# ictnlp/StreamSpeech

Measured on NVIDIA H100. Metric: audio-seconds/sec (RTF^-1) Fr-En simul S2ST @chunk=320ms, higher is better.
Workload: dtype f32

## Files before the change

### include/streamspeech_b200.h

```cpp
#ifndef STREAMSPEECH_B200_H_
#define STREAMSPEECH_B200_H_

#include <stdint.h>

#ifdef __cplusplus
extern "C" {
#endif

typedef struct ss_engine ss_engine;

enum ss_status {
  SS_OK = 0,
  SS_ERR_INVALID = -1,
  SS_ERR_MISSING = -2,
  SS_ERR_CUDA = -3,
  SS_ERR_STATE = -4,
  SS_ERR_CAPACITY = -5
};

#define SS_MAX_UPS 8
#define SS_MAX_RB 4
#define SS_MAX_DIL 4

typedef struct ss_config {
// ... 63 lines not shown
                        float* wav_out_dev);
int ss_vocoder_hop(const ss_engine* h);
int ss_vocoder_receptive_field(const ss_engine* h);

int ss_pool_create(ss_engine* h, int n_slots, int max_seconds);
int ss_pool_create_rate(ss_engine* h, int n_slots, int max_seconds, int sample_rate);
int ss_pool_reset(ss_engine* h, int slot);
int ss_pool_push_audio(ss_engine* h, void* stream, int slot, const float* samples_host, int n);
int ss_pool_finish(ss_engine* h, int slot);
int ss_pool_info(ss_engine* h, int slot, int64_t* n_audio, int32_t* n_feat, int32_t* T_final, float** enc_out_dev, float** feats_dev);
int ss_pool_step(ss_engine* h, void* stream, int n, const int32_t* slots_host, int ctc_heads, int64_t* packed_out_dev, int64_t packed_capacity,
                 int32_t* T_out_host, int32_t* T_final_out_host, int64_t* out_off_host);

int ss_op_linear(ss_engine* h, void* stream, const float* x_dev, int M, int K, const float* w_dev, const float* bias_dev, int N,
                 int act, float* out_dev);
int ss_op_linear_umma(ss_engine* h, void* stream, const float* x_dev, int M, int K, const float* w_dev, const float* bias_dev, int N,
                      int act, int pieces, float* out_dev);
int ss_op_conv1d(ss_engine* h, void* stream, const float* x_dev, int L, int C_in, const float* w_dev, const float* bias_dev, int N,
                 int ksize, int dil, int pad_left, float pre_lrelu, int mode, float* out_dev);
int ss_set_option(ss_engine* h, const char* name, int value);
int ss_debug_copy(ss_engine* h, const char* what, void* host_dst, size_t bytes);
int ss_op_layer_norm(ss_engine* h, void* stream, const float* x_dev, int rows, int C, const float* g_dev, const float* b_dev,
                     float* out_dev);

int64_t ss_launch_count(const ss_engine* h);
int ss_async_error(ss_engine* h);

#ifdef __cplusplus
}
#endif
#endif
```

### streamspeech_b200/csrc/engine.h

```cpp
#pragma once
#include <cuda_runtime.h>

#include <map>
#include <tuple>
#include <utility>
#include <string>
#include <vector>

#include "../../include/streamspeech_b200.h"
#include "kernels.h"
#include "kernels_persist.h"
#include "kernels_multistream.h"

namespace ss {

struct HostTensor {
  std::vector<float> data;
  std::vector<int64_t> shape;
  int64_t numel() const {
    int64_t n = 1;
    for (auto s : shape) n *= s;
    return n;
  }
};
// ... 43 lines not shown
  float* bias = nullptr;
};

struct Arena {
  char* base = nullptr;
  size_t cap = 0, off = 0;
  float* f32(size_t n) { return (float*)raw(n * 4); }
  void* raw(size_t bytes);
  void reset() { off = 0; }
  bool ensure(size_t bytes);
};

}

struct ss_engine {
  int device = 0;
  ss_config cfg{};
  std::string err;
  bool finalized = false;
  int attn_chunk = 8, conv_chunk = 8;
  int umma_vocoder = 0;
  int umma_linear = 0;
  int unit_grouped = 1;
  int umma_min_rows = 128;
  int umma_min_channels = 16;
  ss::Umma2Cache* umma2_cache = nullptr;
  int vocoder_streams = 1;
  cudaStream_t aux_stream[2] = {nullptr, nullptr};
  cudaEvent_t fork_event = nullptr, join_event[2] = {nullptr, nullptr};
  int vocoder_graph = 0;
  int graph_pdl = 0;
  cudaStream_t capture_stream = nullptr;
  std::map<std::tuple<int, uintptr_t, int, int, int>, std::pair<cudaGraphExec_t, int>> voc_graphs;
  int vocoder_fused = -1;
  std::map<std::pair<int, uintptr_t>, ss::VocFusedParams> voc_fused;
  float* persist_ffn_scratch = nullptr;
  float* cl_blobs = nullptr;
  int cluster_cooperative = 1;
  long long cl_steps = 0;
  int persistent_encoder_cluster = 0;
  int persistent_ffn_fused = 1;
  int fbank_tma = 1;
  int persistent_encoder = 1;
  std::map<std::string, ss::HostTensor> host;
  std::vector<void*> dev_allocs;

// ... 103 lines not shown
```

### streamspeech_b200/csrc/engine_run.cu

```cuda
#include <algorithm>
#include <cmath>
#include <cstring>
#include <stdexcept>
#include <tuple>

#include "engine.h"

using namespace ss;

namespace {

inline cudaStream_t S(void* s) { return (cudaStream_t)s; }

int check_launch(ss_engine* h, const char* where) {
  cudaError_t e = cudaGetLastError();
  if (e != cudaSuccess) return h->fail(SS_ERR_CUDA, std::string(where) + ": " + cudaGetErrorString(e));
  return SS_OK;
}

thread_local int g_umma_linear = 0;
thread_local int g_umma_conv = 0;
thread_local int g_umma_min_rows = 128;
thread_local int g_umma_min_channels = 16;
thread_local Umma2Cache* g_umma2_cache = nullptr;
// ... 180 lines not shown
        const float s = m + 1 < nd ? 1.0f : 1.0f / nrb;
        job(rbT[j], nullptr, nullptr, L, L, ch, w2.ksize, 1, (w2.ksize - 1) / 2, 0.1f, w2.lin.w, w2.lin.b, out, ch, 1, 0, cur, s, s);
      }
      phase(first);
    }
  }
  if (!ok || jobs.size() > VOC_MAX_JOBS || phases.size() > VOC_MAX_PHASES || vocoder_fused_smem(a_stride, b_stride) > 200 * 1024) return nullptr;
  if (h->voc_fused.size() >= 64) h->voc_fused.clear();
  VocFusedParams& p = h->voc_fused[key];
  std::copy(jobs.begin(), jobs.end(), p.jobs);
  std::copy(phases.begin(), phases.end(), p.phases);
  p.n_phases = (int)phases.size();
  p.a_stride = a_stride;
  p.b_stride = b_stride;
  return &p;
}

struct DecScratch {
  float *y, *q, *kv, *attn, *hid, *qkv;
};

void dec_layer(const DecLayerW& L, float* x, int n, int dim, int ffn, int heads, bool causal, int self_kv_len_limit,
               const int* self_kv_len_dev, float* cache_k, float* cache_v, int past, const float* cross_kv, int Tk,
               const int* cross_len_dev, DecScratch& s, cudaStream_t st, int group_R = 0, const int* group_len_dev = nullptr) {
  const float scale = 0.125f;
  if (group_R > 1 && !cache_k && causal && n % group_R == 0) {
    const int S = n / group_R;
    ln_linear(x, dim * group_R, S, L.self_ln, L.qkv, ep_out(s.qkv, 3 * dim), s.y, st);
    grouped_causal_attention(s.qkv, 3 * dim, s.qkv + dim, 3 * dim, s.qkv + 2 * dim, 3 * dim, s.attn, dim, S, group_R, heads, scale, group_len_dev, st);
  } else if (cache_k) {
    ln_qkv_routed(x, dim, n, L.self_ln, L.qkv, dim, s.q, dim, cache_k + (size_t)past * dim, dim, cache_v + (size_t)past * dim, dim, s.y, st);
    mha_attention(s.q, dim, cache_k, dim, cache_v, dim, s.attn, dim, 1, n, past + n, heads, scale, 1, past, self_kv_len_dev, st);
  } else {
    ln_linear(x, dim, n, L.self_ln, L.qkv, ep_out(s.qkv, 3 * dim), s.y, st);
    mha_attention(s.qkv, 3 * dim, s.qkv + dim, 3 * dim, s.qkv + 2 * dim, 3 * dim, s.attn, dim, 1, n, n, heads, scale,
                  causal ? 1 : 0, 0, self_kv_len_dev, st);
  }
  (void)self_kv_len_limit;
  linear(s.attn, dim, n, L.out, ep_residual(x, dim), st);
  if (L.has_cross) {
    ln_linear(x, dim, n, L.cross_ln, L.cq, ep_out(s.q, dim), s.y, st);
    mha_attention(s.q, dim, cross_kv, 2 * dim, cross_kv + dim, 2 * dim, s.attn, dim, 1, n, Tk, heads, scale, 0, 0, cross_len_dev, st);
    linear(s.attn, dim, n, L.cout, ep_residual(x, dim), st);
  }
  ln_linear(x, dim, n, L.final_ln, L.fc1, ep_out(s.hid, ffn, ACT_RELU), s.y, st);
  linear(s.hid, ffn, n, L.fc2, ep_residual(x, dim), st);
}

int ensure_mt_cross(ss_engine* h, int T, int keep_rows = 0) {
  if (T <= h->mt_cross_cap) return SS_OK;
  const int cap = std::max(T + T / 2, 512);
  const size_t row = (size_t)2 * h->cfg.mt_dim;
  float* fresh = nullptr;
  if (cudaMalloc((void**)&fresh, (size_t)h->cfg.mt_layers * cap * row * sizeof(float)) != cudaSuccess) return h->fail(SS_ERR_CUDA, "cudaMalloc(mt cross kv) failed");
  if (h->mt_cross_kv) {
    cudaDeviceSynchronize();
    if (keep_rows > 0)
      for (int l = 0; l < h->cfg.mt_layers; ++l)
        cudaMemcpy(fresh + (size_t)l * cap * row, h->mt_cross_kv + (size_t)l * h->mt_cross_cap * row, (size_t)keep_rows * row * sizeof(float), cudaMemcpyDeviceToDevice);
// ... 636 lines not shown
  float* t2u = t2u_out_dev ? t2u_out_dev : h->ws.f32((size_t)Slen * dim);
  int* kvlen = nullptr;
  int* kvlen_up = nullptr;
  if (n_pad_tail > 0) {
    int v[2] = {Slen - n_pad_tail, (Slen - n_pad_tail) * R};
    kvlen = (int*)h->ws.raw(2 * sizeof(int));
    kvlen_up = kvlen + 1;
    cudaMemcpyAsync(kvlen, v, sizeof(v), cudaMemcpyHostToDevice, st);
    cudaStreamSynchronize(st);
  }
  copy_f32(mt_feats_dev, x, (int64_t)Slen * dim, st);
  for (int l = 0; l < c.t2u_layers; ++l)
    dec_layer(h->t2u[l], x, Slen, dim, c.unit_ffn, c.unit_heads, c.uni_encoder != 0, 0, kvlen, nullptr, nullptr, 0, nullptr, 0, nullptr, s1, st);
  layer_norm(x, dim, t2u, dim, h->t2u_ln.g, h->t2u_ln.b, Slen, dim, st);
  DecScratch s2 = dec_scratch(h, L, dim, c.unit_ffn);
  float* xu = h->ws.f32((size_t)L * dim);
  float* ckv = h->ws.f32((size_t)Slen * 2 * dim);
  float* logits = logits_dev ? logits_dev : h->ws.f32((size_t)L * c.unit_vocab);
  if (!xu || !ckv || !logits) return h->fail(SS_ERR_CUDA, "workspace too small");
  repeat_rows_add(t2u, Slen, R, dim, h->unit_pos_row, xu, st);
  for (int l = 0; l < c.unit_layers; ++l) {
    linear(t2u, dim, Slen, h->unit[l].ckv, ep_out(ckv, 2 * dim), st);
    const int gR = (l == 0 && h->unit_grouped) ? R : 0;
    dec_layer(h->unit[l], xu, L, dim, c.unit_ffn, c.unit_heads, true, 0, kvlen_up, nullptr, nullptr, 0, ckv, Slen, kvlen, s2, st, gR, kvlen);
  }
  layer_norm(xu, dim, xu, dim, h->unit_ln.g, h->unit_ln.b, L, dim, st);
  Linear outp;
  outp.w = h->unit_emb; outp.b = nullptr; outp.N = c.unit_vocab; outp.K = dim;
  linear(xu, dim, L, outp, ep_out(logits, c.unit_vocab), st);
  argmax_rows(logits, c.unit_vocab, L, c.unit_vocab, h->mask_pad_unk, mask_eos ? 3 : 2, argmax_dev, nullptr, st);
  ctc_collapse(argmax_dev, L, c.unit_vocab - 1, c.pad, units_dev, nullptr, count_dev, st);
  return check_launch(h, "ss_t2u_unit_decode");
}

int ss_unit_position_row(ss_engine* h, const float* row_host) {
  if (!h || !h->finalized || !row_host) return h ? h->fail(SS_ERR_STATE, "engine not finalized / null row") : SS_ERR_INVALID;
  cudaDeviceSynchronize();
  if (cudaMemcpy(h->unit_pos_row, row_host, (size_t)h->cfg.unit_dim * sizeof(float), cudaMemcpyHostToDevice) != cudaSuccess)
    return h->fail(SS_ERR_CUDA, "cudaMemcpy(unit positional row) failed");
  return SS_OK;
}

int ss_vocoder_durations(ss_engine* h, void* stream, const int64_t* codes_dev, int U, int dur_prediction, int64_t* dur_out_dev,
                         int32_t* cumsum_out_dev) {
  if (!h || !h->finalized) return h ? h->fail(SS_ERR_STATE, "engine not finalized") : SS_ERR_INVALID;
  if (!h->has_vocoder) return h->fail(SS_ERR_STATE, "no vocoder weights were loaded");
  if (U <= 0) return h->fail(SS_ERR_INVALID, "empty code sequence");
// ... 239 lines not shown
  if (n == "umma_vocoder") h->umma_vocoder = value;
  else if (n == "umma_linear") h->umma_linear = value;
  else if (n == "umma_min_rows") h->umma_min_rows = value;
  else if (n == "umma_min_channels") h->umma_min_channels = value;
  else if (n == "umma2_cache_clear") {
    umma2_cache_clear(h->umma2_cache);
    clear_graphs(h);
  }
  else if (n == "umma2_split_below") { g_umma2_split_below = value; clear_graphs(h); }
  else if (n == "umma2_min_units") { g_umma2_min_units = value; clear_graphs(h); }
  else if (n == "umma2_debug") {
    if (value && !g_umma2_dbg) {
      if (cudaMalloc(&g_umma2_dbg, 16 * sizeof(unsigned long long)) != cudaSuccess) return h->fail(SS_ERR_CUDA, "cudaMalloc failed");
      cudaMemset(g_umma2_dbg, 0, 16 * sizeof(unsigned long long));
    }
    if (!value && g_umma2_dbg) {
      cudaDeviceSynchronize();
      cudaFree(g_umma2_dbg);
      g_umma2_dbg = nullptr;
    }
  }
  else if (n == "prefer_shared") g_prefer_shared = value;
  else if (n == "unit_grouped") h->unit_grouped = value;
  else if (n == "vocoder_graph") h->vocoder_graph = value;
  else if (n == "vocoder_fused") h->vocoder_fused = value;
  else if (n == "graph_pdl") h->graph_pdl = value;
  else if (n == "fbank_tma") h->fbank_tma = value;
  else if (n == "umma2_fused_reduce") g_umma2_fused_reduce = value;
  else if (n == "persistent_encoder") h->persistent_encoder = value;
  else if (n == "persistent_ffn_fused") h->persistent_ffn_fused = value;
  else if (n == "cluster_cooperative") h->cluster_cooperative = value;
  else if (n == "persistent_encoder_cluster") {
    if (value && !h->cl_blobs) {
      if (!h->persist_layers || !h->persist_bar) return h->fail(SS_ERR_STATE, "persistent_encoder_cluster needs a finalized engine");
      const size_t n_f = encoder_layers_cluster_blob_floats(h->cfg.enc_layers);
      if (h->cfg.enc_dim != 256 || h->cfg.enc_ffn != 2048) return h->fail(SS_ERR_INVALID, "persistent_encoder_cluster: encoder must be 256 / 2048");
      if (cudaMalloc(&h->cl_blobs, n_f * sizeof(float)) != cudaSuccess) return h->fail(SS_ERR_CUDA, "cudaMalloc failed");
      h->dev_allocs.push_back(h->cl_blobs);
      encoder_layers_cluster_pack(h->persist_layers, h->cfg.enc_layers, h->cfg.dw_kernel, h->cl_blobs, 0);
      if (cudaDeviceSynchronize() != cudaSuccess) return h->fail(SS_ERR_CUDA, "packing the cluster weight blobs failed");
    }
    h->persistent_encoder_cluster = value;
  }
  else if (n == "vocoder_streams") h->vocoder_streams = value;
  else if (n == "persistent_mt") h->persistent_mt = value;
  else if (n == "persistent_mt_prefix") h->persistent_mt_prefix = value;
// ... 118 lines not shown
  } else if (mode >= 2) {
    return h->fail(SS_ERR_INVALID, "modes 2 / 3 (first-generation tensor-core kernel) were removed: use 12 / 13");
  } else {
    gemm_conv(a, w_dev, N, ep, S(stream));
  }
  return check_launch(h, "ss_op_conv1d");
}

int ss_op_linear(ss_engine* h, void* stream, const float* x_dev, int M, int K, const float* w_dev, const float* bias_dev, int N, int act,
                 float* out_dev) {
  if (!h) return SS_ERR_INVALID;
  Linear l;
  l.w = const_cast<float*>(w_dev); l.b = const_cast<float*>(bias_dev); l.N = N; l.K = K;
  linear(x_dev, K, M, l, ep_out(out_dev, N, act), S(stream));
  return check_launch(h, "ss_op_linear");
}

int ss_op_layer_norm(ss_engine* h, void* stream, const float* x_dev, int rows, int C, const float* g_dev, const float* b_dev, float* out_dev) {
  if (!h) return SS_ERR_INVALID;
  layer_norm(x_dev, C, out_dev, C, g_dev, b_dev, rows, C, S(stream));
  return check_launch(h, "ss_op_layer_norm");
}

}

#include "engine_pool.inc"
```

### streamspeech_b200/csrc/kernels.h

```cpp
#pragma once
#include <cuda_runtime.h>
#include <stdint.h>

namespace ss {

extern unsigned long long g_launches;
extern int g_prefer_shared;
extern thread_local int g_pdl_off;

enum Act : int { ACT_NONE = 0, ACT_RELU = 1, ACT_SILU = 2, ACT_TANH = 3 };

struct ConvA {
  const float* x = nullptr;
  int B = 1;
  int L_in = 0;
  int L_rows = 0;
  int C_in = 0;
  int ldx = 0;
  int ksize = 1;
  int stride = 1;
  int dil = 1;
  int pad_left = 0;
  int chunk = 0;
  float pre_lrelu = 1.0f;
// ... 78 lines not shown
int vocoder_fused(const VocFusedParams& p, unsigned* bar_ctr, unsigned* bar_target_host, cudaStream_t st);

bool skinny_gemm_supported(int M, int N, int K, const Epilogue& ep);
void skinny_gemm(const float* A, int lda, const float* W, int M, int N, int K, const Epilogue& ep, cudaStream_t st);

void layer_norm(const float* x, int ldx, float* y, int ldy, const float* gamma, const float* beta, int rows, int C,
                cudaStream_t st);

void fbank_cmvn(const float* samples, int64_t n_samples, int f0, int nf, const float* mel_bank ,
                const float* window , const float* cmvn_mean, const float* cmvn_inv_std_or_null,
                const float* cmvn_std, float* out , cudaStream_t st);

void fbank_cmvn_tma(const float* samples, int f0, int nf, const float* melT, const float* window, const float* cmvn_mean, const float* cmvn_std,
                    float* out, cudaStream_t st);

void relpos_attention(const float* q, int ldq, const float* k, int ldk, const float* v, int ldv, const float* pos, int Tpos,
                      const float* bias_u, const float* bias_v, float* out, int B, int nQ, int q_offset, int T, int H, int D,
                      int chunk , const int* lengths_dev, cudaStream_t st);

void mha_attention(const float* q, int ldq, const float* k, int ldk, const float* v, int ldv, float* out, int ldo, int B,
                   int Tq, int Tk, int H, float scale, int causal, int causal_offset, const int* kv_len_dev,
                   cudaStream_t st);

void grouped_causal_attention(const float* q, int ldq, const float* k, int ldk, const float* v, int ldv, float* out, int ldo, int S, int R,
                              int H, float scale, const int* kv_len_dev, cudaStream_t st);

void depthwise_bn_silu(const float* x, int ldx, const float* w , const float* scale, const float* shift,
                       float* y, int ldy, int B, int T, int t0, int n, int C, int k, int chunk, cudaStream_t st);

void scale_rows(float* x, int64_t n, float s, cudaStream_t st);
void embed_tokens_pos(const int64_t* tokens, const int* positions_or_null, int pos_offset, const float* emb,
                      const float* pos_table, float scale, float* out, int rows, int C, int pad_idx, cudaStream_t st);
void repeat_rows_add(const float* x, int S, int R, int C, const float* addvec_or_null, float* out, cudaStream_t st);
void argmax_rows(const float* logits, int ld, int rows, int V, const int* masked_cols, int n_masked, int64_t* out_idx,
                 float* out_lprob_or_null, cudaStream_t st);
void ctc_collapse(const int64_t* argmax, int n, int blank, int pad, int64_t* out_tokens, int* out_index, int* out_count,
                  cudaStream_t st);
void ctc_argmax_collapse_pair(const float* logits, int ld, int V, int n_new, int row0, int n_rows, const int* masked, int n_masked, int blank,
                              int pad, int64_t* am0, int64_t* am1, int64_t* out, int out_stride, unsigned* ticket, cudaStream_t st);
void gather_rows(const int64_t* idx, int n, int idx_offset, const float* table, int C, float* out, cudaStream_t st);
void duration_from_log(const float* logdur, int n, int64_t* dur, int* cumsum , cudaStream_t st);
void expand_frames(const float* emb , const int* cumsum , int U, int f0, int nf, int C, float* out,
                   cudaStream_t st);
void conv_post_tanh(const float* x, int L, int C, const float* w , float bias, int k, float pre_slope, float* out,
                    cudaStream_t st);
void copy_f32(const float* src, float* dst, int64_t n, cudaStream_t st);
// ... 5 lines not shown
```

### streamspeech_b200/csrc/kernels_attn.cu

```cuda
#include "common.cuh"
#include "kernels.h"

namespace ss {
namespace {

constexpr int QT = 16;
constexpr int KT = 64;
constexpr int ATT_NT = 128;
constexpr int HD = 64;
constexpr int LDK = HD + 4;

__device__ __forceinline__ float dot64(const float* __restrict__ a, const float* __restrict__ b) {
  float acc = 0.f;
#pragma unroll
  for (int d = 0; d < HD; d += 4) {
    float4 x = *reinterpret_cast<const float4*>(a + d);
    float4 y = *reinterpret_cast<const float4*>(b + d);
    acc = fmaf(x.x, y.x, acc);
    acc = fmaf(x.y, y.y, acc);
    acc = fmaf(x.z, y.z, acc);
    acc = fmaf(x.w, y.w, acc);
  }
  return acc;
}
// ... 262 lines not shown
    float e = expf(smem[j] - mx);
    smem[j] = e;
    if (j < n_prev) sum += e;
  }
  sum = block_sum128(sum, red);
  __syncthreads();
  {
    const int d = threadIdx.x & (HD - 1), half = threadIdx.x >> 6;
    float a = 0.f;
    for (int j = half; j < n_prev; j += 2) a = fmaf(smem[j], v[(int64_t)j * ldv + h * HD + d], a);
    part[half][d] = a;
  }
  __syncthreads();
  const float e_own = own ? smem[n_prev] : 0.f;
  for (int idx = threadIdx.x; idx < R * HD; idx += ATT_NT) {
    const int r = idx >> 6, d = idx & (HD - 1);
    const float c = own ? (float)(r + 1) : 0.f;
    const float num = (float)R * (part[0][d] + part[1][d]) + c * e_own * (own ? v[(int64_t)g * ldv + h * HD + d] : 0.f);
    const float den = (float)R * sum + c * e_own;
    out[((int64_t)g * R + r) * ldo + h * HD + d] = num / den;
  }
}

template <bool RELPOS>
void launch_attn(const float* q, int ldq, const float* k, int ldk, const float* v, int ldv, const float* pos, int Tpos, int ldp,
                 const float* bias_u, const float* bias_v, float* out, int ldo, int B, int nQ, int q_offset, int T, int H, float scale,
                 int chunk, int causal, int causal_offset, const int* lengths, cudaStream_t st) {
  const long tiles = (long)((nQ + QT - 1) / QT) * H * B;
  if (tiles < 96 && (size_t)T * sizeof(float) <= 160 * 1024) {
    size_t smem_row = (size_t)((T + 3) & ~3) * sizeof(float);
    if (smem_row > 40 * 1024 && first_time_on_device((const void*)attn_row_kernel<RELPOS>))
      cudaFuncSetAttribute(attn_row_kernel<RELPOS>, cudaFuncAttributeMaxDynamicSharedMemorySize, 160 * 1024);
    launch_pdl(attn_row_kernel<RELPOS>, dim3(dim3(nQ, H, B)), dim3(ATT_NT), smem_row, st, q, ldq, k, ldk, v, ldv, pos, Tpos, ldp, bias_u, bias_v, out, ldo, nQ,
                                                                      q_offset, T, scale, chunk, causal, causal_offset, lengths);
    return;
  }
  size_t smem = (size_t)((RELPOS ? 2 : 1) * QT * LDK + 2 * KT * LDK + (RELPOS ? (KT + QT - 1) * LDK : 0) + QT * (KT + 1)) * sizeof(float);
  if (first_time_on_device((const void*)attn_tile_kernel<RELPOS>))
    cudaFuncSetAttribute(attn_tile_kernel<RELPOS>, cudaFuncAttributeMaxDynamicSharedMemorySize, (int)smem);
  launch_pdl(attn_tile_kernel<RELPOS>, dim3(dim3((nQ + QT - 1) / QT, H, B)), dim3(ATT_NT), smem, st, q, ldq, k, ldk, v, ldv, pos, Tpos, ldp, bias_u, bias_v, out, ldo,
                                                                                 nQ, q_offset, T, scale, chunk, causal, causal_offset, lengths);
}

}

void relpos_attention(const float* q, int ldq, const float* k, int ldk, const float* v, int ldv, const float* pos, int Tpos,
                      const float* bias_u, const float* bias_v, float* out, int B, int nQ, int q_offset, int T, int H, int D,
                      int chunk, const int* lengths_dev, cudaStream_t st) {
  ++g_launches;
  if (B <= 0 || T <= 0 || nQ <= 0) return;
  launch_attn<true>(q, ldq, k, ldk, v, ldv, pos, Tpos, D, bias_u, bias_v, out, D, B, nQ, q_offset, T, H, 0.125f, chunk, 0, 0, lengths_dev, st);
}

void grouped_causal_attention(const float* q, int ldq, const float* k, int ldk, const float* v, int ldv, float* out, int ldo, int S, int R,
                              int H, float scale, const int* kv_len_dev, cudaStream_t st) {
  ++g_launches;
  if (S <= 0 || R <= 0) return;
  launch_pdl(grouped_causal_attn_kernel, dim3(S, H), dim3(ATT_NT), (size_t)((S + 3) & ~3) * sizeof(float), st, q, ldq, k, ldk, v, ldv, out, ldo, S, R,
             scale, kv_len_dev);
}

void mha_attention(const float* q, int ldq, const float* k, int ldk, const float* v, int ldv, float* out, int ldo, int B,
                   int Tq, int Tk, int H, float scale, int causal, int causal_offset, const int* kv_len_dev,
                   cudaStream_t st) {
  ++g_launches;
  if (B <= 0 || Tq <= 0 || Tk <= 0) return;
  launch_attn<false>(q, ldq, k, ldk, v, ldv, nullptr, 0, 0, nullptr, nullptr, out, ldo, B, Tq, 0, Tk, H, scale, 0, causal, causal_offset,
                     kv_len_dev, st);
}

}
```

### streamspeech_b200/engine.py

```python
from __future__ import annotations

import ctypes
import os
from typing import Dict, List, Optional, Sequence, Tuple

import torch

from . import constants
from .config import ModelConfig

_HERE = os.path.dirname(os.path.abspath(__file__))
LIB_PATH = os.path.join(_HERE, "libstreamspeech_b200.so")
SS_MAX_UPS, SS_MAX_RB, SS_MAX_DIL = 8, 4, 4


class SSConfig(ctypes.Structure):
    _fields_ = (
        [(n, ctypes.c_int32) for n in (
            "feat_dim", "enc_dim", "enc_ffn", "enc_heads", "enc_layers", "dw_kernel", "conv_channels", "conv_kernel",
            "src_vocab", "tgt_vocab", "mt_dim", "mt_ffn", "mt_heads", "mt_layers",
            "t2u_layers", "unit_dim", "unit_ffn", "unit_heads", "unit_layers", "unit_vocab", "ctc_upsample_rate",
            "bos", "pad", "eos", "unk", "uni_encoder", "max_enc_frames", "max_mt_positions", "voc_n_ups")]
        + [("voc_up_rates", ctypes.c_int32 * SS_MAX_UPS), ("voc_up_kernels", ctypes.c_int32 * SS_MAX_UPS),
           ("voc_init_channels", ctypes.c_int32), ("voc_n_rb", ctypes.c_int32),
# ... 34 lines not shown
    lib.ss_fbank.argtypes = [vp, vp, vp, i64, i64, i64, vp]
    lib.ss_encoder_forward.argtypes = [vp, vp, vp, vp, i32, i32, vp]
    lib.ss_encoder_stream_reset.argtypes = [vp]
    lib.ss_encoder_stream_step.argtypes = [vp, vp, vp, i32, vp, ctypes.POINTER(i32), ctypes.POINTER(i32)]
    lib.ss_ctc_greedy.argtypes = [vp, vp, i32, vp, i32, vp, vp, vp, vp]
    lib.ss_ctc_greedy_rows.argtypes = [vp, vp, i32, vp, i32, i32, vp, vp, vp, vp]
    lib.ss_ctc_greedy_pair.argtypes = [vp, vp, vp, i32, i32, vp, vp, vp]
    lib.ss_mt_greedy.argtypes = [vp, vp, vp, i32, vp, i32, i32, i32, vp, i32, ctypes.POINTER(i32), vp]
    lib.ss_mt_stable_rows.argtypes = [vp, i32]
    lib.ss_mt_incremental_reset.argtypes = [vp]
    lib.ss_mt_greedy_incremental.argtypes = [vp, vp, vp, i32, vp, i32, i32, i32, vp, i32, ctypes.POINTER(i32)]
    lib.ss_mt_features.argtypes = [vp, vp, vp, i32, vp, i32, vp, vp]
    lib.ss_t2u_unit_decode.argtypes = [vp, vp, vp, i32, i32, i32, vp, vp, vp, vp, vp]
    lib.ss_unit_position_row.argtypes = [vp, vp]
    lib.ss_vocoder_durations.argtypes = [vp, vp, vp, i32, i32, vp, vp]
    lib.ss_vocoder_generate.argtypes = [vp, vp, i32, i32, i32, i32, vp]
    lib.ss_vocoder_hop.argtypes = [vp]
    lib.ss_vocoder_receptive_field.argtypes = [vp]
    lib.ss_op_linear.argtypes = [vp, vp, vp, i32, i32, vp, vp, i32, i32, vp]
    lib.ss_op_linear_umma.argtypes = [vp, vp, vp, i32, i32, vp, vp, i32, i32, i32, vp]
    lib.ss_op_conv1d.argtypes = [vp, vp, vp, i32, i32, vp, vp, i32, i32, i32, i32, ctypes.c_float, i32, vp]
    lib.ss_set_option.argtypes = [vp, ctypes.c_char_p, i32]
    lib.ss_op_layer_norm.argtypes = [vp, vp, vp, i32, i32, vp, vp, vp]
    lib.ss_debug_copy.argtypes = [vp, ctypes.c_char_p, vp, ctypes.c_size_t]
    lib.ss_launch_count.argtypes = [vp]
    lib.ss_launch_count.restype = i64
    lib.ss_async_error.argtypes = [vp]
    lib.ss_resample_out_len.argtypes = [i64, i32]
    lib.ss_resample_out_len.restype = i64
    lib.ss_resample_48k_to_16k.argtypes = [vp, vp, vp, i64, i64, i64, vp]
    lib.ss_pool_create.argtypes = [vp, i32, i32]
    lib.ss_pool_create_rate.argtypes = [vp, i32, i32, i32]
    lib.ss_pool_reset.argtypes = [vp, i32]
    lib.ss_pool_finish.argtypes = [vp, i32]
    lib.ss_pool_push_audio.argtypes = [vp, vp, i32, vp, i32]
    lib.ss_pool_info.argtypes = [vp, i32, ctypes.POINTER(i64), ctypes.POINTER(i32), ctypes.POINTER(i32), ctypes.POINTER(vp), ctypes.POINTER(vp)]
    lib.ss_pool_step.argtypes = [vp, vp, i32, vp, i32, vp, i64, vp, vp, vp]
    _lib = lib
    return lib


EXPORTED_SYMBOLS = [
    "ss_create", "ss_destroy", "ss_last_error", "ss_version", "ss_load_tensor", "ss_finalize", "ss_set_chunk",
    "ss_fbank_num_frames", "ss_fbank", "ss_encoder_out_frames", "ss_encoder_forward", "ss_encoder_stream_reset", "ss_encoder_stream_step", "ss_ctc_greedy", "ss_ctc_greedy_rows", "ss_mt_greedy",
    "ss_mt_features", "ss_mt_stable_rows", "ss_t2u_unit_decode", "ss_unit_position_row", "ss_vocoder_durations", "ss_vocoder_generate", "ss_vocoder_hop",
    "ss_vocoder_receptive_field", "ss_op_linear", "ss_op_linear_umma", "ss_op_conv1d", "ss_set_option", "ss_debug_copy", "ss_op_layer_norm", "ss_launch_count", "ss_async_error", "ss_mt_incremental_reset", "ss_mt_greedy_incremental", "ss_ctc_greedy_pair", "ss_resample_out_len", "ss_resample_48k_to_16k", "ss_pool_create", "ss_pool_reset", "ss_pool_push_audio", "ss_pool_info", "ss_pool_step",
    "ss_pool_create_rate", "ss_pool_finish",
]


def make_ss_config(cfg: ModelConfig, max_enc_frames: int, max_mt_positions: int = 1024) -> SSConfig:
    c = SSConfig()
    for n in ("feat_dim", "enc_dim", "enc_ffn", "enc_heads", "enc_layers", "dw_kernel", "conv_channels", "conv_kernel",
              "src_vocab", "tgt_vocab", "mt_dim", "mt_ffn", "mt_heads", "mt_layers", "t2u_layers", "unit_dim", "unit_ffn",
              "unit_heads", "unit_layers", "unit_vocab", "ctc_upsample_rate", "bos", "pad", "eos", "unk"):
        setattr(c, n, int(getattr(cfg, n)))
    c.uni_encoder = int(cfg.uni_encoder)
    c.max_enc_frames = max_enc_frames
    c.max_mt_positions = max_mt_positions
    v = cfg.vocoder
    c.voc_n_ups = len(v.upsample_rates)
    for i, (u, k) in enumerate(zip(v.upsample_rates, v.upsample_kernel_sizes)):
        c.voc_up_rates[i], c.voc_up_kernels[i] = u, k
    c.voc_init_channels = v.upsample_initial_channel
    c.voc_n_rb = len(v.resblock_kernel_sizes)
    c.voc_rb_ndil = len(v.resblock_dilation_sizes[0])
    for j, (k, dils) in enumerate(zip(v.resblock_kernel_sizes, v.resblock_dilation_sizes)):
        c.voc_rb_kernels[j] = k
        assert len(dils) == c.voc_rb_ndil
        for m, d in enumerate(dils):
# ... 46 lines not shown
            if gcmvn is not None:
                self._load("__const__.gcmvn_mean", torch.as_tensor(gcmvn["mean"], dtype=torch.float32))
                self._load("__const__.gcmvn_std", torch.as_tensor(gcmvn["std"], dtype=torch.float32))
            self._check(self.lib.ss_finalize(self._h))
        except Exception:
            self.close()
            raise
        self.set_option("prefer_shared", int(os.environ.get("SS_PREFER_SHARED", "0")))
        self.set_option("umma_vocoder", int(os.environ.get("SS_UMMA_VOCODER", "12")))
        self.set_option("umma_linear", int(os.environ.get("SS_UMMA_LINEAR", "13")))
        self.set_option("umma_min_rows", int(os.environ.get("SS_UMMA_MIN_ROWS", "128")))
        self.set_option("umma_min_channels", int(os.environ.get("SS_UMMA_MIN_CHANNELS", "16")))
        self.set_option("persistent_encoder", int(os.environ.get("SS_PERSISTENT_ENCODER", "1")))
        self.set_option("persistent_mt", int(os.environ.get("SS_PERSISTENT_MT", "1")))
        self.set_option("umma2_fused_reduce", int(os.environ.get("SS_UMMA2_FUSED_REDUCE", "0")))
        self.set_option("fbank_tma", int(os.environ.get("SS_FBANK_TMA", "1")))
        self.set_option("persistent_ffn_fused", int(os.environ.get("SS_PERSISTENT_FFN_FUSED", "1")))
        self.set_option("persistent_encoder_cluster", int(os.environ.get("SS_PERSISTENT_ENCODER_CLUSTER", "1")))
        self.set_option("cluster_cooperative", int(os.environ.get("SS_CLUSTER_COOPERATIVE", "1")))
        self.set_option("persistent_mt_v2", int(os.environ.get("SS_PERSISTENT_MT_V2", "1")))
        self.set_option("persistent_mt_prefix", int(os.environ.get("SS_PERSISTENT_MT_PREFIX", "1")))
        self.set_option("vocoder_streams", int(os.environ.get("SS_VOCODER_STREAMS", "1")))
        self.set_option("unit_grouped", int(os.environ.get("SS_UNIT_GROUPED", "1")))
        self.set_option("vocoder_graph", int(os.environ.get("SS_VOCODER_GRAPH", "0")))
        self.set_option("vocoder_fused", int(os.environ.get("SS_VOCODER_FUSED", "-1")))
        self.set_option("graph_pdl", int(os.environ.get("SS_GRAPH_PDL", "0")))
        self.set_option("persistent_prefetch", int(os.environ.get("SS_PERSISTENT_PREFETCH", "0")))
        self.set_option("umma2_split_below", int(os.environ.get("SS_UMMA2_SPLIT_BELOW", "60")))
        self.set_option("umma2_min_units", int(os.environ.get("SS_UMMA2_MIN_UNITS", "4")))
        self.set_option("persistent_barrier", int(os.environ.get("SS_PERSISTENT_BARRIER", "1")))
        self.hop = self.lib.ss_vocoder_hop(self._h)
        self.vocoder_receptive_field = self.lib.ss_vocoder_receptive_field(self._h)

    def close(self):
        if getattr(self, "_h", None) is not None and self._h:
            self.lib.ss_destroy(self._h)
            self._h = None

    def __del__(self):
        try:
            self.close()
        except Exception:
            pass

    def _check(self, rc: int):
        if rc != 0:
# ... 270 lines not shown
        sl = (ctypes.c_int32 * n)(*[int(x) for x in slots])
        T, Tf, off = (ctypes.c_int32 * n)(), (ctypes.c_int32 * n)(), (ctypes.c_int64 * n)()
        self._check(self.lib.ss_pool_step(self._h, self._stream(), n, sl, int(ctc_heads), self._pool_out.data_ptr(), self._pool_out.numel(), T, Tf, off))
        res = [{"T": int(T[i]), "T_final": int(Tf[i]), "ctc": []} for i in range(n)]
        if ctc_heads:
            used = int(off[n - 1]) + ctc_heads * (2 * int(T[n - 1]) + 2)
            host = self._pool_out[:used].cpu()
            for i in range(n):
                Ti = int(T[i])
                for hd in range(ctc_heads):
                    o = int(off[i]) + hd * (2 * Ti + 2)
                    row = host[o:o + 2 * Ti + 2]
                    cnt = int(row[:1].view(torch.int32)[0])
                    res[i]["ctc"].append((row[1:1 + cnt].tolist(), row[1 + Ti:].view(torch.int32)[:cnt].tolist()))
        return res

    def set_option(self, name: str, value: int):
        self._check(self.lib.ss_set_option(self._h, name.encode(), int(value)))

    def op_layer_norm(self, x: torch.Tensor, g: torch.Tensor, b: torch.Tensor) -> torch.Tensor:
        out = torch.empty_like(x)
        self._check(self.lib.ss_op_layer_norm(self._h, self._stream(), x.data_ptr(), x.shape[0], x.shape[1], g.data_ptr(), b.data_ptr(), out.data_ptr()))
        return out
```

Baseline: 133.0.

## Add tensor-core flash causal attention for unit decoder self-attention

Adds a flash-style causal self-attention kernel built on bf16 mma.sync. It splits each fp32 value into three bf16 parts and runs six products per tile, so accuracy stays close to fp32. The kernel is used in the unit decoder's non-grouped layers behind a new option that is on by default, replacing the scalar mha_attention path. It also exposes a standalone op for testing. The three-way split roughly multiplies tensor-core work and adds conversion overhead in exchange for using the MMA units instead of CUDA-core FMAs.

```diff
diff --git a/include/streamspeech_b200.h b/include/streamspeech_b200.h
--- a/include/streamspeech_b200.h
+++ b/include/streamspeech_b200.h
@@ -109,6 +109,8 @@
 int ss_debug_copy(ss_engine* h, const char* what, void* host_dst, size_t bytes);
 int ss_op_layer_norm(ss_engine* h, void* stream, const float* x_dev, int rows, int C, const float* g_dev, const float* b_dev,
                      float* out_dev);
+int ss_op_causal_attention(ss_engine* h, void* stream, const float* qkv_dev, int T, int H, const int* kv_len_dev, int tensor_cores,
+                           float* out_dev);
 
 int64_t ss_launch_count(const ss_engine* h);
 int ss_async_error(ss_engine* h);
diff --git a/streamspeech_b200/csrc/engine.h b/streamspeech_b200/csrc/engine.h
--- a/streamspeech_b200/csrc/engine.h
+++ b/streamspeech_b200/csrc/engine.h
@@ -89,6 +89,7 @@
   int umma_vocoder = 0;
   int umma_linear = 0;
   int unit_grouped = 1;
+  int unit_decoder_v2 = 1;
   int umma_min_rows = 128;
   int umma_min_channels = 16;
   ss::Umma2Cache* umma2_cache = nullptr;
diff --git a/streamspeech_b200/csrc/engine_run.cu b/streamspeech_b200/csrc/engine_run.cu
--- a/streamspeech_b200/csrc/engine_run.cu
+++ b/streamspeech_b200/csrc/engine_run.cu
@@ -226,7 +226,8 @@
 
 void dec_layer(const DecLayerW& L, float* x, int n, int dim, int ffn, int heads, bool causal, int self_kv_len_limit,
                const int* self_kv_len_dev, float* cache_k, float* cache_v, int past, const float* cross_kv, int Tk,
-               const int* cross_len_dev, DecScratch& s, cudaStream_t st, int group_R = 0, const int* group_len_dev = nullptr) {
+               const int* cross_len_dev, DecScratch& s, cudaStream_t st, int group_R = 0, const int* group_len_dev = nullptr,
+               bool tc_self_attn = false) {
   const float scale = 0.125f;
   if (group_R > 1 && !cache_k && causal && n % group_R == 0) {
     const int S = n / group_R;
@@ -237,8 +238,12 @@
     mha_attention(s.q, dim, cache_k, dim, cache_v, dim, s.attn, dim, 1, n, past + n, heads, scale, 1, past, self_kv_len_dev, st);
   } else {
     ln_linear(x, dim, n, L.self_ln, L.qkv, ep_out(s.qkv, 3 * dim), s.y, st);
-    mha_attention(s.qkv, 3 * dim, s.qkv + dim, 3 * dim, s.qkv + 2 * dim, 3 * dim, s.attn, dim, 1, n, n, heads, scale,
-                  causal ? 1 : 0, 0, self_kv_len_dev, st);
+    if (tc_self_attn && causal && dim == heads * 64 &&
+        causal_attention_mma_supported(s.qkv, 3 * dim, s.qkv + dim, 3 * dim, s.qkv + 2 * dim, 3 * dim, s.attn, dim))
+      causal_attention_mma(s.qkv, 3 * dim, s.qkv + dim, 3 * dim, s.qkv + 2 * dim, 3 * dim, s.attn, dim, n, heads, scale, self_kv_len_dev, st);
+    else
+      mha_attention(s.qkv, 3 * dim, s.qkv + dim, 3 * dim, s.qkv + 2 * dim, 3 * dim, s.attn, dim, 1, n, n, heads, scale,
+                    causal ? 1 : 0, 0, self_kv_len_dev, st);
   }
   (void)self_kv_len_limit;
   linear(s.attn, dim, n, L.out, ep_residual(x, dim), st);
@@ -921,7 +926,8 @@
   for (int l = 0; l < c.unit_layers; ++l) {
     linear(t2u, dim, Slen, h->unit[l].ckv, ep_out(ckv, 2 * dim), st);
     const int gR = (l == 0 && h->unit_grouped) ? R : 0;
-    dec_layer(h->unit[l], xu, L, dim, c.unit_ffn, c.unit_heads, true, 0, kvlen_up, nullptr, nullptr, 0, ckv, Slen, kvlen, s2, st, gR, kvlen);
+    dec_layer(h->unit[l], xu, L, dim, c.unit_ffn, c.unit_heads, true, 0, kvlen_up, nullptr, nullptr, 0, ckv, Slen, kvlen, s2, st, gR, kvlen,
+              h->unit_decoder_v2 != 0);
   }
   layer_norm(xu, dim, xu, dim, h->unit_ln.g, h->unit_ln.b, L, dim, st);
   Linear outp;
@@ -1207,6 +1213,7 @@
   }
   else if (n == "prefer_shared") g_prefer_shared = value;
   else if (n == "unit_grouped") h->unit_grouped = value;
+  else if (n == "unit_decoder_v2") h->unit_decoder_v2 = value;
   else if (n == "vocoder_graph") h->vocoder_graph = value;
   else if (n == "vocoder_fused") h->vocoder_fused = value;
   else if (n == "graph_pdl") h->graph_pdl = value;
@@ -1371,6 +1378,19 @@
   return check_launch(h, "ss_op_layer_norm");
 }
 
+int ss_op_causal_attention(ss_engine* h, void* stream, const float* qkv_dev, int T, int H, const int* kv_len_dev, int tensor_cores, float* out_dev) {
+  if (!h || !qkv_dev || !out_dev || T <= 0 || H <= 0) return h ? h->fail(SS_ERR_INVALID, "ss_op_causal_attention: bad arguments") : SS_ERR_INVALID;
+  const int D = H * 64;
+  if (tensor_cores) {
+    if (!causal_attention_mma_supported(qkv_dev, 3 * D, qkv_dev + D, 3 * D, qkv_dev + 2 * D, 3 * D, out_dev, D))
+      return h->fail(SS_ERR_INVALID, "ss_op_causal_attention: misaligned buffers");
+    causal_attention_mma(qkv_dev, 3 * D, qkv_dev + D, 3 * D, qkv_dev + 2 * D, 3 * D, out_dev, D, T, H, 0.125f, kv_len_dev, S(stream));
+  } else {
+    mha_attention(qkv_dev, 3 * D, qkv_dev + D, 3 * D, qkv_dev + 2 * D, 3 * D, out_dev, D, 1, T, T, H, 0.125f, 1, 0, kv_len_dev, S(stream));
+  }
+  return check_launch(h, "ss_op_causal_attention");
+}
+
 }
 
 #include "engine_pool.inc"
diff --git a/streamspeech_b200/csrc/kernels.h b/streamspeech_b200/csrc/kernels.h
--- a/streamspeech_b200/csrc/kernels.h
+++ b/streamspeech_b200/csrc/kernels.h
@@ -124,6 +124,10 @@
                    int Tq, int Tk, int H, float scale, int causal, int causal_offset, const int* kv_len_dev,
                    cudaStream_t st);
 
+bool causal_attention_mma_supported(const float* q, int ldq, const float* k, int ldk, const float* v, int ldv, const float* out, int ldo);
+void causal_attention_mma(const float* q, int ldq, const float* k, int ldk, const float* v, int ldv, float* out, int ldo, int T, int H,
+                          float scale, const int* kv_len_dev, cudaStream_t st);
+
 void grouped_causal_attention(const float* q, int ldq, const float* k, int ldk, const float* v, int ldv, float* out, int ldo, int S, int R,
                               int H, float scale, const int* kv_len_dev, cudaStream_t st);
 
diff --git a/streamspeech_b200/csrc/kernels_attn.cu b/streamspeech_b200/csrc/kernels_attn.cu
--- a/streamspeech_b200/csrc/kernels_attn.cu
+++ b/streamspeech_b200/csrc/kernels_attn.cu
@@ -1,3 +1,5 @@
+#include <cuda_bf16.h>
+
 #include "common.cuh"
 #include "kernels.h"
 
@@ -308,6 +310,212 @@
   }
 }
 
+constexpr int TC_QT = 64;
+constexpr int TC_KT = 64;
+constexpr int TC_P = HD + 8;
+constexpr int TC_FP = HD + 4;
+constexpr int TC_SMEM = 2 * 3 * TC_KT * TC_P * 2 + 2 * TC_KT * TC_FP * 4;
+
+__device__ __forceinline__ void cp_async16_zfill(float* dst, const float* src, bool ok) {
+  asm volatile("cp.async.cg.shared.global [%0], [%1], 16, %2;" ::"r"((uint32_t)__cvta_generic_to_shared(dst)), "l"(src), "r"(ok ? 16 : 0)
+               : "memory");
+}
+
+__device__ __forceinline__ void split3_bf16x2(float x, float y, uint32_t (&o)[3]) {
+#pragma unroll
+  for (int p = 0; p < 3; ++p) {
+    __nv_bfloat162 hv = __floats2bfloat162_rn(x, y);
+    o[p] = *reinterpret_cast<uint32_t*>(&hv);
+    x -= __low2float(hv);
+    y -= __high2float(hv);
+  }
+}
+
+__device__ __forceinline__ void mma_bf16_16816(float (&d)[4], const uint32_t (&a)[4], uint32_t b0, uint32_t b1) {
+  asm volatile("mma.sync.aligned.m16n8k16.row.col.f32.bf16.bf16.f32 {%0, %1, %2, %3}, {%4, %5, %6, %7}, {%8, %9}, {%0, %1, %2, %3};"
+               : "+f"(d[0]), "+f"(d[1]), "+f"(d[2]), "+f"(d[3])
+               : "r"(a[0]), "r"(a[1]), "r"(a[2]), "r"(a[3]), "r"(b0), "r"(b1));
+}
+
+__device__ __forceinline__ void mma_split6(float (&d)[4], const uint32_t (&a)[3][4], const uint32_t (&b)[3][2]) {
+  mma_bf16_16816(d, a[2], b[0][0], b[0][1]);
+  mma_bf16_16816(d, a[0], b[2][0], b[2][1]);
+  mma_bf16_16816(d, a[1], b[1][0], b[1][1]);
+  mma_bf16_16816(d, a[1], b[0][0], b[0][1]);
+  mma_bf16_16816(d, a[0], b[1][0], b[1][1]);
+  mma_bf16_16816(d, a[0], b[0][0], b[0][1]);
+}
+
+__global__ void __launch_bounds__(ATT_NT, 2) causal_attn_mma_kernel(const float* __restrict__ q, int ldq, const float* __restrict__ k, int ldk,
+                                                                    const float* __restrict__ v, int ldv, float* __restrict__ out, int ldo, int T,
+                                                                    float scale, const int* __restrict__ kv_len) {
+  pdl_trigger();
+  pdl_wait();
+  extern __shared__ __align__(16) unsigned char smem_tc[];
+  __nv_bfloat16* Ks = reinterpret_cast<__nv_bfloat16*>(smem_tc);
+  __nv_bfloat16* Vt = Ks + 3 * TC_KT * TC_P;
+  float* Kf = reinterpret_cast<float*>(Vt + 3 * HD * TC_P);
+  float* Vf = Kf + TC_KT * TC_FP;
+  const int h = blockIdx.y;
+  const int q0 = (gridDim.x - 1 - blockIdx.x) * TC_QT;
+  const int warp = threadIdx.x >> 5, lane = threadIdx.x & 31, g = lane >> 2, c = lane & 3;
+  const int len = kv_len ? min(kv_len[0], T) : T;
+  const int rw = q0 + warp * 16;
+  auto nvis = [&](int i) { return max(1, min(i + 1, len)); };
+  const int kmax_cta = nvis(min(q0 + TC_QT, T) - 1);
+  const int kmax_w = rw < T ? nvis(min(rw + 15, T - 1)) : 0;
+  const int lim[2] = {nvis(rw + g), nvis(rw + g + 8)};
+  const float* kb = k + h * HD;
+  const float* vb = v + h * HD;
+
+  uint32_t qa[4][3][4];
+#pragma unroll
+  for (int ks = 0; ks < 4; ++ks)
+#pragma unroll
+    for (int r = 0; r < 4; ++r) {
+      const int row = rw + g + 8 * (r & 1);
+      float2 x = make_float2(0.f, 0.f);
+      if (row < T) x = *reinterpret_cast<const float2*>(q + (int64_t)row * ldq + h * HD + 16 * ks + 8 * (r >> 1) + 2 * c);
+      uint32_t w[3];
+      split3_bf16x2(x.x * scale, x.y * scale, w);
+#pragma unroll
+      for (int p = 0; p < 3; ++p) qa[ks][p][r] = w[p];
+    }
+  float o[8][4];
+#pragma unroll
+  for (int nt = 0; nt < 8; ++nt)
+#pragma unroll
+    for (int e = 0; e < 4; ++e) o[nt][e] = 0.f;
+  float m_run[2] = {-INFINITY, -INFINITY}, l_run[2] = {0.f, 0.f};
+
+  auto fetch = [&](int j0) {
+    for (int e = threadIdx.x; e < TC_KT * (HD / 4); e += ATT_NT) {
+      const int r = e >> 4, cc = (e & 15) << 2;
+      const bool ok = j0 + r < kmax_cta;
+      const int64_t row = ok ? j0 + r : 0;
+      cp_async16_zfill(Kf + r * TC_FP + cc, kb + row * ldk + cc, ok);
+      cp_async16_zfill(Vf + r * TC_FP + cc, vb + row * ldv + cc, ok);
+    }
+    asm volatile("cp.async.commit_group;" ::: "memory");
+  };
+  fetch(0);
+  for (int j0 = 0; j0 < kmax_cta; j0 += TC_KT) {
+    asm volatile("cp.async.wait_group 0;" ::: "memory");
+    __syncthreads();
+    for (int e = threadIdx.x; e < TC_KT * (HD / 4); e += ATT_NT) {
+      const int r = e >> 4, cc = (e & 15) << 2;
+      const float4 x = *reinterpret_cast<const float4*>(Kf + r * TC_FP + cc);
+      uint32_t lo[3], hi[3];
+      split3_bf16x2(x.x, x.y, lo);
+      split3_bf16x2(x.z, x.w, hi);
+#pragma unroll
+      for (int p = 0; p < 3; ++p) *reinterpret_cast<uint2*>(Ks + (p * TC_KT + r) * TC_P + cc) = make_uint2(lo[p], hi[p]);
+    }
+    for (int e = threadIdx.x; e < (TC_KT / 2) * (HD / 4); e += ATT_NT) {
+      const int kp = e & 31, d0 = (e >> 5) << 2;
+      const float4 a = *reinterpret_cast<const float4*>(Vf + 2 * kp * TC_FP + d0);
+      const float4 b = *reinterpret_cast<const float4*>(Vf + (2 * kp + 1) * TC_FP + d0);
+      const float av[4] = {a.x, a.y, a.z, a.w}, bv[4] = {b.x, b.y, b.z, b.w};
+#pragma unroll
+      for (int t = 0; t < 4; ++t) {
+        uint32_t w[3];
+        split3_bf16x2(av[t], bv[t], w);
+#pragma unroll
+        for (int p = 0; p < 3; ++p) *reinterpret_cast<uint32_t*>(Vt + (p * HD + d0 + t) * TC_P + 2 * kp) = w[p];
+      }
+    }
+    __syncthreads();
+    if (j0 + TC_KT < kmax_cta) fetch(j0 + TC_KT);
+    if (j0 >= kmax_w) continue;
+
+    float s[8][4];
+#pragma unroll
+    for (int nt = 0; nt < 8; ++nt) {
+#pragma unroll
+      for (int e = 0; e < 4; ++e) s[nt][e] = 0.f;
+#pragma unroll
+      for (int ks = 0; ks < 4; ++ks) {
+        uint32_t b[3][2];
+#pragma unroll
+        for (int p = 0; p < 3; ++p) {
+          const __nv_bfloat16* kr = Ks + (p * TC_KT + 8 * nt + g) * TC_P + 16 * ks + 2 * c;
+          b[p][0] = *reinterpret_cast<const uint32_t*>(kr);
+          b[p][1] = *reinterpret_cast<const uint32_t*>(kr + 8);
+        }
+        mma_split6(s[nt], qa[ks], b);
+      }
+    }
+#pragma unroll
+    for (int rh = 0; rh < 2; ++rh) {
+      float mx = -INFINITY;
+#pragma unroll
+      for (int nt = 0; nt < 8; ++nt)
+#pragma unroll
+        for (int e = 0; e < 2; ++e) {
+          const int j = j0 + 8 * nt + 2 * c + e;
+          if (j >= lim[rh]) s[nt][2 * rh + e] = -INFINITY;
+          mx = fmaxf(mx, s[nt][2 * rh + e]);
+        }
+      mx = fmaxf(mx, __shfl_xor_sync(0xffffffffu, mx, 1));
+      mx = fmaxf(mx, __shfl_xor_sync(0xffffffffu, mx, 2));
+      const float m_new = fmaxf(m_run[rh], mx);
+      const float corr = (m_new == -INFINITY) ? 1.f : expf(m_run[rh] - m_new);
+      float sum = 0.f;
+#pragma unroll
+      for (int nt = 0; nt < 8; ++nt)
+#pragma unroll
+        for (int e = 0; e < 2; ++e) {
+          const float sv = s[nt][2 * rh + e];
+          const float pv = (sv == -INFINITY) ? 0.f : expf(sv - m_new);
+          s[nt][2 * rh + e] = pv;
+          sum += pv;
+        }
+      sum += __shfl_xor_sync(0xffffffffu, sum, 1);
+      sum += __shfl_xor_sync(0xffffffffu, sum, 2);
+      l_run[rh] = l_run[rh] * corr + sum;
+      m_run[rh] = m_new;
+#pragma unroll
+      for (int nt = 0; nt < 8; ++nt) {
+        o[nt][2 * rh] *= corr;
+        o[nt][2 * rh + 1] *= corr;
+      }
+    }
+#pragma unroll
+    for (int kk = 0; kk < 4; ++kk) {
+      uint32_t pa[3][4];
+#pragma unroll
+      for (int r = 0; r < 4; ++r) {
+        uint32_t w[3];
+        const float* sv = s[2 * kk + (r >> 1)];
+        split3_bf16x2(sv[2 * (r & 1)], sv[2 * (r & 1) + 1], w);
+#pragma unroll
+        for (int p = 0; p < 3; ++p) pa[p][r] = w[p];
+      }
+#pragma unroll
+      for (int nt = 0; nt < 8; ++nt) {
+        uint32_t b[3][2];
+#pragma unroll
+        for (int p = 0; p < 3; ++p) {
+          const __nv_bfloat16* vr = Vt + (p * HD + 8 * nt + g) * TC_P + 16 * kk + 2 * c;
+          b[p][0] = *reinterpret_cast<const uint32_t*>(vr);
+          b[p][1] = *reinterpret_cast<const uint32_t*>(vr + 8);
+        }
+        mma_split6(o[nt], pa, b);
+      }
+    }
+  }
+#pragma unroll
+  for (int rh = 0; rh < 2; ++rh) {
+    const int row = rw + g + 8 * rh;
+    if (row < T) {
+      const float inv = 1.0f / l_run[rh];
+      float* op = out + (int64_t)row * ldo + h * HD + 2 * c;
+#pragma unroll
+      for (int nt = 0; nt < 8; ++nt) *reinterpret_cast<float2*>(op + 8 * nt) = make_float2(o[nt][2 * rh] * inv, o[nt][2 * rh + 1] * inv);
+    }
+  }
+}
+
 template <bool RELPOS>
 void launch_attn(const float* q, int ldq, const float* k, int ldk, const float* v, int ldv, const float* pos, int Tpos, int ldp,
                  const float* bias_u, const float* bias_v, float* out, int ldo, int B, int nQ, int q_offset, int T, int H, float scale,
@@ -346,6 +554,22 @@
              scale, kv_len_dev);
 }
 
+bool causal_attention_mma_supported(const float* q, int ldq, const float* k, int ldk, const float* v, int ldv, const float* out, int ldo) {
+  const auto aligned = [](const float* p, uintptr_t bytes) { return (reinterpret_cast<uintptr_t>(p) & (bytes - 1)) == 0; };
+  return (ldq & 1) == 0 && (ldo & 1) == 0 && (ldk & 3) == 0 && (ldv & 3) == 0 && aligned(k, 16) && aligned(v, 16) && aligned(q, 8) &&
+         aligned(out, 8);
+}
+
+void causal_attention_mma(const float* q, int ldq, const float* k, int ldk, const float* v, int ldv, float* out, int ldo, int T, int H,
+                          float scale, const int* kv_len_dev, cudaStream_t st) {
+  ++g_launches;
+  if (T <= 0) return;
+  if (first_time_on_device((const void*)causal_attn_mma_kernel))
+    cudaFuncSetAttribute(causal_attn_mma_kernel, cudaFuncAttributeMaxDynamicSharedMemorySize, TC_SMEM);
+  launch_pdl(causal_attn_mma_kernel, dim3((T + TC_QT - 1) / TC_QT, H), dim3(ATT_NT), (size_t)TC_SMEM, st, q, ldq, k, ldk, v, ldv, out, ldo, T,
+             scale, kv_len_dev);
+}
+
 void mha_attention(const float* q, int ldq, const float* k, int ldk, const float* v, int ldv, float* out, int ldo, int B,
                    int Tq, int Tk, int H, float scale, int causal, int causal_offset, const int* kv_len_dev,
                    cudaStream_t st) {
diff --git a/streamspeech_b200/engine.py b/streamspeech_b200/engine.py
--- a/streamspeech_b200/engine.py
+++ b/streamspeech_b200/engine.py
@@ -80,6 +80,7 @@
     lib.ss_op_conv1d.argtypes = [vp, vp, vp, i32, i32, vp, vp, i32, i32, i32, i32, ctypes.c_float, i32, vp]
     lib.ss_set_option.argtypes = [vp, ctypes.c_char_p, i32]
     lib.ss_op_layer_norm.argtypes = [vp, vp, vp, i32, i32, vp, vp, vp]
+    lib.ss_op_causal_attention.argtypes = [vp, vp, vp, i32, i32, vp, i32, vp]
     lib.ss_debug_copy.argtypes = [vp, ctypes.c_char_p, vp, ctypes.c_size_t]
     lib.ss_launch_count.argtypes = [vp]
     lib.ss_launch_count.restype = i64
@@ -103,7 +104,7 @@
     "ss_fbank_num_frames", "ss_fbank", "ss_encoder_out_frames", "ss_encoder_forward", "ss_encoder_stream_reset", "ss_encoder_stream_step", "ss_ctc_greedy", "ss_ctc_greedy_rows", "ss_mt_greedy",
     "ss_mt_features", "ss_mt_stable_rows", "ss_t2u_unit_decode", "ss_unit_position_row", "ss_vocoder_durations", "ss_vocoder_generate", "ss_vocoder_hop",
     "ss_vocoder_receptive_field", "ss_op_linear", "ss_op_linear_umma", "ss_op_conv1d", "ss_set_option", "ss_debug_copy", "ss_op_layer_norm", "ss_launch_count", "ss_async_error", "ss_mt_incremental_reset", "ss_mt_greedy_incremental", "ss_ctc_greedy_pair", "ss_resample_out_len", "ss_resample_48k_to_16k", "ss_pool_create", "ss_pool_reset", "ss_pool_push_audio", "ss_pool_info", "ss_pool_step",
-    "ss_pool_create_rate", "ss_pool_finish",
+    "ss_pool_create_rate", "ss_pool_finish", "ss_op_causal_attention",
 ]
 
 
@@ -196,6 +197,7 @@
         self.set_option("persistent_mt_prefix", int(os.environ.get("SS_PERSISTENT_MT_PREFIX", "1")))
         self.set_option("vocoder_streams", int(os.environ.get("SS_VOCODER_STREAMS", "1")))
         self.set_option("unit_grouped", int(os.environ.get("SS_UNIT_GROUPED", "1")))
+        self.set_option("unit_decoder_v2", int(os.environ.get("SS_UNIT_DECODER_V2", "1")))
         self.set_option("vocoder_graph", int(os.environ.get("SS_VOCODER_GRAPH", "0")))
         self.set_option("vocoder_fused", int(os.environ.get("SS_VOCODER_FUSED", "-1")))
         self.set_option("graph_pdl", int(os.environ.get("SS_GRAPH_PDL", "0")))
@@ -512,3 +514,11 @@
         out = torch.empty_like(x)
         self._check(self.lib.ss_op_layer_norm(self._h, self._stream(), x.data_ptr(), x.shape[0], x.shape[1], g.data_ptr(), b.data_ptr(), out.data_ptr()))
         return out
+
+    def op_causal_attention(self, qkv: torch.Tensor, heads: int, kv_len: Optional[int] = None, tensor_cores: bool = True) -> torch.Tensor:
+        assert qkv.is_cuda and qkv.dtype == torch.float32 and qkv.is_contiguous() and qkv.shape[1] == 3 * heads * 64
+        T = qkv.shape[0]
+        out = self._f32(T, heads * 64)
+        kl = None if kv_len is None else torch.tensor([int(kv_len)], dtype=torch.int32, device=self.device)
+        self._check(self.lib.ss_op_causal_attention(self._h, self._stream(), qkv.data_ptr(), T, heads, self._ptr(kl), int(tensor_cores), out.data_ptr()))
+        return out
```

New measurement: 136.2 (median of 6 runs). 1.02x the previous value.
